# fritzsedlazeck/Sniffles

Hardware: NVIDIA H100
Metric: aligned long-read Gbp/s through lead->cluster->consensus (higher is better)
Workload: dtype int32

## Files before the change

### sniffles_b200/csrc/api.cu

```cuda
#include <algorithm>
#include <climits>
#include <cstdio>
#include <cstdlib>
#include <cstring>
#include <string>
#include <vector>
#include <dlfcn.h>
#include <omp.h>

#include "common.cuh"
#include "prims.cuh"
#include "extract.cuh"
#include "cluster.cuh"
#include "consensus.cuh"
#include "poa.cuh"
#include "combine.cuh"
#include "population.cuh"
#include "ingest.cuh"
#include "bgzf_write.cuh"
#include "genotype.cuh"
#include "rnames.cuh"
#include "reference.cuh"

template <bool Pinned> struct Buf {
// ... 786 lines not shown
    mark(ctx, "kept_bins");
    prims::exclusive_scan(ctx->launches, b.bin_nl, b.kl_off, b.scan_tmp, &ctr->n_bins, nb, &ctr->n_kl, st);
    prims::exclusive_scan(ctx->launches, b.bin_nlong, b.kll_off, b.scan_tmp, &ctr->n_bins, nb, &ctr->n_kll, st);
    prims::exclusive_scan(ctx->launches, b.bin_kept, b.kb_idx, b.scan_tmp, &ctr->n_bins, nb, &ctr->n_kbins, st);
    launch(ctx->launches, cluster::k_kbin_build, g, 128, 0, st, b);
    launch(ctx->launches, cluster::k_gather_kept, grid_for(nb, 256), 256, 0, st, b);
    mark(ctx, "merge_chains");
    launch(ctx->launches, cluster::k_seg_heads, g, 128, 0, st, b);
    prims::exclusive_scan(ctx->launches, b.flag, b.scan, b.scan_tmp, &ctr->n_kbins, nb, &ctr->n_segs, st);
    launch(ctx->launches, cluster::k_seg_build, g, 128, 0, st, b);
    launch(ctx->launches, cluster::k_merge, g, 128, 0, st, b);
    launch(ctx->launches, cluster::k_verify_cuts, g, 128, 0, st, b);
    prims::exclusive_scan(ctx->launches, b.flag, b.scan, b.scan_tmp, &ctr->n_kbins, nb, &ctr->n_clusters, st);
    launch(ctx->launches, cluster::k_cluster_build, g, 128, 0, st, b);
    mark(ctx, "cluster_call");
    CUDA_TRY(cudaEventRecord(ctx->ev_fork, st)); CUDA_TRY(cudaStreamWaitEvent(ctx->st_side, ctx->ev_fork, 0));
    launch(ctx->launches, cluster::k_cluster_block, NUM_SMS, cluster::CB_THREADS, cluster::CB_SMEM, ctx->st_side, b);
    launch(ctx->launches, cluster::k_cluster_warp<cluster::WARP_CAP, cluster::CWM_WARPS, true>, NUM_SMS * 2, cluster::CWM_WARPS * 32, cluster::CwCfg<cluster::WARP_CAP, cluster::CWM_WARPS>::smem, ctx->st_side, b);
    CUDA_TRY(cudaEventRecord(ctx->ev_join, ctx->st_side));
    launch(ctx->launches, cluster::k_cluster_warp<cluster::SMALL_CAP, cluster::CWS_WARPS, false>, NUM_SMS * 4, cluster::CWS_WARPS * 32, cluster::CwCfg<cluster::SMALL_CAP, cluster::CWS_WARPS>::smem, st, b);
    CUDA_TRY(cudaStreamWaitEvent(st, ctx->ev_join, 0));
    mark(ctx, "emit_cands");
    prims::exclusive_scan(ctx->launches, b.cl_nvalid, b.cl_cand_base, b.scan_tmp, &ctr->n_clusters, nb, &ctr->n_cand, st);
    prims::exclusive_scan(ctx->launches, b.cl_nlead, b.cl_lead_base, b.scan_tmp, &ctr->n_clusters, nb, &ctr->n_cand_leads, st);
    prims::exclusive_scan(ctx->launches, b.cl_nrn, b.cl_rn_base, b.scan_tmp, &ctr->n_clusters, nb, &ctr->n_rnames, st);
    launch(ctx->launches, cluster::k_emit_cands, NUM_SMS * 8, 128, 0, st, b);
    mark(ctx, "coverage");
    if (ctx->n_mask) launch(ctx->launches, cluster::k_mask_bp, grid_for((unsigned long long)ctx->n_mask * 32, 128), 128, 0, st, b, ctx->b_mask_task.as<uint32_t>(), ctx->n_mask, ctx->task_cov);
    launch(ctx->launches, cluster::k_coverage, NUM_SMS * 32, 128, 0, st, b);
    consensus::C& c = ctx->Cc;
    CUDA_TRY(cudaMemsetAsync(c.work, 0, sizeof(consensus::Work), st));
    mark(ctx, "consensus_plan");
    launch(ctx->launches, consensus::k_plan, grid_for(ctx->cap.cand, 128), 128, 0, st, c);
    prims::exclusive_scan(ctx->launches, c.alt_len, c.alt_off, b.scan_tmp, &ctr->n_cand, ctx->cap.cand, &ctr->n_alt_bytes, st);
    prims::exclusive_scan(ctx->launches, c.scr_len, c.scr_off, b.scan_tmp, &ctr->n_cand, ctx->cap.cand, &ctr->n_seq_bytes, st);
    prims::exclusive_scan_cols(ctx->launches, c.q_cnt, c.q_off, ctx->cap.cand + 1, consensus::NQ, ctx->q_scan_tmp, &ctr->n_cand, ctx->cap.cand, c.work->n, st);
    launch(ctx->launches, consensus::k_plan_finish, grid_for(ctx->cap.cand, 128), 128, 0, st, c);
    launch(ctx->launches, consensus::k_plan_slices, 1, 32, 0, st, c, ctx->n_slices);
    mark(ctx, nullptr);
    CUDA_TRY(cudaGetLastError());
    return 0;
}

static int enqueue_stage_c(snfb_ctx* ctx) {
    cluster::B& b = ctx->B; consensus::C& c = ctx->Cc; DevCounters* ctr = b.ctr; cudaStream_t st = ctx->st;
    c.seq = ctx->d_seq; c.arena_off = nullptr; ctx->seq_h2d_bytes = 0;
    if (ctx->seq_on_demand) {
        mark(ctx, "seq_requests");
        launch(ctx->launches, consensus::k_seq_requests, grid_for(ctx->cap.cand, 128), 128, 0, st, c, ctx->seq_req, ctx->cap.req, ctx->arena_off, &ctr->n_req, &ctr->n_req_units);
        mark(ctx, nullptr);
        CUDA_TRY(cudaMemcpyAsync(ctx->h_fin, ctr, sizeof(DevCounters), cudaMemcpyDeviceToHost, st));
        CUDA_TRY(cudaStreamSynchronize(st));
        const unsigned long long nreq = ctx->h_fin->n_req, nunits = ctx->h_fin->n_req_units;
        if (nreq <= ctx->cap.req && nunits <= ctx->cap.req16 && nreq) {
            if (ctx->h_seq_req.ensure(sizeof(consensus::SeqReq) * (nreq + 1)) || ctx->h_seq_arena.ensure(nunits * 16 + 64)) return fail(ctx, "out of pinned memory (seq arena)");
            CUDA_TRY(cudaMemcpyAsync(ctx->h_seq_req.p, ctx->seq_req, sizeof(consensus::SeqReq) * nreq, cudaMemcpyDeviceToHost, st));
            CUDA_TRY(cudaStreamSynchronize(st));
            const consensus::SeqReq* rq = ctx->h_seq_req.as<consensus::SeqReq>(); uint8_t* dst = ctx->h_seq_arena.as<uint8_t>(); const uint8_t* src = ctx->h_seq; const uint64_t nseq = ctx->n_seq;
            #pragma omp parallel for schedule(static, 256)
            for (long long i = 0; i < (long long)nreq; ++i) {
                unsigned long long s0 = rq[i].src; unsigned long long nbytes = rq[i].nbytes; if (s0 > nseq) s0 = nseq; if (s0 + nbytes > nseq) nbytes = nseq - s0;
                memcpy(dst + (size_t)rq[i].dst16 * 16, src + s0, (size_t)nbytes);
            }
            mark(ctx, "h2d_seq_slices", nunits * 16);
            CUDA_TRY(cudaMemcpyAsync(ctx->seq_arena, ctx->h_seq_arena.p, nunits * 16, cudaMemcpyHostToDevice, st));
            mark(ctx, nullptr);
            ctx->seq_h2d_bytes = nunits * 16;
        }
        c.seq = ctx->seq_arena; c.arena_off = ctx->arena_off;
    }
    CUDA_TRY(cudaEventRecord(ctx->ev_fork, st)); CUDA_TRY(cudaStreamWaitEvent(ctx->st_side, ctx->ev_fork, 0));
    for (int s = 0; s < ctx->n_slices; ++s) {
        cudaStream_t ss = (s & 1) ? ctx->st_side : st; const bool on_main = ss == st;
        if (s) CUDA_TRY(cudaStreamWaitEvent(ss, ctx->ev_aligned[s - 1], 0));
        if (on_main) mark(ctx, "consensus");
        launch(ctx->launches, consensus::k_prep, NUM_SMS * 8, 128, 0, ss, c, s);
        if (on_main) mark(ctx, "consensus_align");
        launch(ctx->launches, consensus::k_align, NUM_SMS * 7, consensus::ALIGN_WARPS * 32, 0, ss, c, s);
        CUDA_TRY(cudaEventRecord(ctx->ev_aligned[s], ss));
        if (on_main) mark(ctx, "consensus_vote");
        launch(ctx->launches, consensus::k_vote, NUM_SMS * 16, consensus::VOTE_THREADS, 0, ss, c, s);
        CUDA_TRY(cudaEventRecord(ctx->ev_slice[s], ss));
    }
    CUDA_TRY(cudaEventRecord(ctx->ev_join, ctx->st_side)); CUDA_TRY(cudaStreamWaitEvent(st, ctx->ev_join, 0));
    mark(ctx, nullptr);
    CUDA_TRY(cudaGetLastError());
    return 0;
}

static void initial_caps(snfb_ctx* ctx) {
    Caps& k = ctx->cap;
    const unsigned long long nrec = ctx->n_rec;
    const unsigned long long lead = std::max<unsigned long long>(1ull << 16, nrec) + (unsigned long long)extract::WALK_BLOCKS * (extract::WALK_THREADS / 32) * extract::WALK_SLOTS
                                    + (unsigned long long)extract::SA_BLOCKS * extract::SA_THREADS * extract::SLOT_CHUNK / 4;
    if (k.lead < lead) k.lead = lead;
    if (k.cand < k.lead / 8 + 1024) k.cand = k.lead / 8 + 1024;
    if (k.cand_lead < k.lead / 2 + 1024) k.cand_lead = k.lead / 2 + 1024;
    if (k.rn < k.lead / 2 + 1024) k.rn = k.lead / 2 + 1024;
    if (k.alt < (4ull << 20)) k.alt = 4ull << 20;
    if (k.scr16 < (2ull << 20)) k.scr16 = 2ull << 20;
    if (k.item < k.cand_lead / 2 + 1024) k.item = k.cand_lead / 2 + 1024;
    if (k.tile < k.cand + 4096) k.tile = k.cand + 4096;
    if (ctx->seq_on_demand) { if (k.req < k.cand_lead / 2 + 1024) k.req = k.cand_lead / 2 + 1024; if (k.req16 < (1ull << 20)) k.req16 = 1ull << 20; }
    else { if (k.req < 16) k.req = 16; if (k.req16 < 16) k.req16 = 16; }
}
static unsigned long long grown(unsigned long long need) { return need + need / 4 + 1024; }
static bool caps_fit(snfb_ctx* ctx, const DevCounters& c, const consensus::Work& work, int upto) {
// ... 821 lines not shown
```

### sniffles_b200/csrc/consensus.cuh

```cuda
#pragma once
#include "common.cuh"

namespace consensus {

constexpr int THREADS = 128;
constexpr int TAB = 2048;
constexpr uint8_t DASH = 0xff;
constexpr int MAXHIT = 512, MAXHIT_LIGHT = 384; constexpr uint32_t HEAVY_L = 3000;

enum { Q_BIG, Q_SMALL, Q_HEAVY, Q_LIGHT, Q_TILE, NQ };
constexpr int MAX_SLICES = 8, DEFAULT_SLICES = 2;
struct Slice { uint32_t c_lo, c_hi; uint32_t lo[NQ], hi[NQ]; unsigned long long alt_lo, alt_hi; };
struct Work {
    unsigned long long n[NQ];
    uint32_t pos[MAX_SLICES][4];
    Slice slice[MAX_SLICES];
};

struct C {
    const snfb_cand* cand; snfb_cand* cand_rw; const snfb_lead* cand_leads;
    const uint32_t* out_plo; const uint32_t* out_pn;
    const uint32_t* ord; const snfb_lead* kleads;
    const snfb_rec* rec; const uint8_t* seq;
    const uint32_t* arena_off;
    uint32_t* plan_best; uint32_t* plan_nother; uint32_t* plan_otot; uint32_t* alt_len; uint32_t* scr_len; uint32_t* alt_off; uint32_t* scr_off;
    uint8_t* alt; uint8_t* scr; unsigned long long alt_cap, scr_cap16, cand_cap;
    uint32_t* work_big; uint32_t* work_small; Work* work;
    uint32_t* q_cnt; uint32_t* q_off;
    struct Item { uint32_t cand; uint32_t k; uint32_t row; uint32_t rd_off; };
    Item* items_big; Item* items_small; uint2* tiles; unsigned long long item_cap, tile_cap;
    DevCounters* ctr; snfb_config cfg;
};

__device__ __forceinline__ uint8_t seq_code(const uint8_t* sq, long long q) { const uint8_t v = sq[q >> 1]; return (q & 1) ? (v & 15) : (v >> 4); }

__global__ void k_plan(C c) {
    const unsigned long long nc = c.ctr->n_cand < c.cand_cap ? c.ctr->n_cand : c.cand_cap;
    for (unsigned long long i = blockIdx.x * (unsigned long long)blockDim.x + threadIdx.x; i < nc; i += (unsigned long long)gridDim.x * blockDim.x) {
        uint32_t al = 0, sl = 0, heavy_n = 0, light_n = 0, tiles = 0; bool big = false;
        if (c.cand[i].svtype == SNFB_INS && !c.cfg.symbolic) {
            const snfb_cand* cd = &c.cand[i]; long nm = 0, bi = -1; long long bd = 0; long long tot = 0;
            for (int k = 0; k < cd->lead_n; ++k) { const snfb_lead* l = &c.cand_leads[cd->lead_off + k]; if (!(l->flags & SNFB_LF_HAS_SEQ)) continue;
                long long a = (long long)l->seq_len - cd->svlen; if (a < 0) a = -a; long long p = (long long)l->ref_start - cd->pos; if (p < 0) p = -p;
                const long long d = 2 * a + 3 * p; if (nm == 0 || d < bd) { bd = d; bi = k; } ++nm; tot += ((long long)l->seq_len + 7) & ~7ll; }
            if (nm > 0) {
                const uint32_t L = (uint32_t)c.cand_leads[cd->lead_off + bi].seq_len; al = L;
                const bool cons = (nm - 1 >= c.cfg.consensus_min_reads) && !c.cfg.no_consensus;
                c.plan_best[i] = (uint32_t)bi; c.plan_nother[i] = cons ? (uint32_t)(nm - 1) : 0u; c.plan_otot[i] = (uint32_t)(tot - ((L + 7u) & ~7u));
                const unsigned long long bytes = cons ? (unsigned long long)tot + 8 + (unsigned long long)(nm - 1) * ((L + 3u) & ~3u) + (unsigned long long)(nm - 1) * 16 + 64 + 16 + TAB * 8 : (unsigned long long)L + 24;
                sl = (uint32_t)((bytes + 15) / 16);
                c.cand_rw[i].alt_len = (int)L;
                big = (unsigned long long)L * (unsigned long long)nm > 60000ull;
                if (cons) { const bool heavy = L > HEAVY_L; heavy_n = heavy ? (uint32_t)(nm - 1) : 0u; light_n = heavy ? 0u : (uint32_t)(nm - 1); tiles = (L + 4095u) / 4096u; }
            }
        }
        c.alt_len[i] = al; c.scr_len[i] = sl;
        const size_t col = c.cand_cap + 1;
        c.q_cnt[Q_BIG * col + i] = sl && big; c.q_cnt[Q_SMALL * col + i] = sl && !big; c.q_cnt[Q_HEAVY * col + i] = heavy_n; c.q_cnt[Q_LIGHT * col + i] = light_n; c.q_cnt[Q_TILE * col + i] = tiles;
    }
}

__global__ void k_plan_finish(C c) {
    const unsigned long long nc = c.ctr->n_cand < c.cand_cap ? c.ctr->n_cand : c.cand_cap; const size_t col = c.cand_cap + 1;
    for (unsigned long long i = blockIdx.x * (unsigned long long)blockDim.x + threadIdx.x; i < nc; i += (unsigned long long)gridDim.x * blockDim.x) {
        if (!c.scr_len[i]) continue;
        c.cand_rw[i].alt_off = (int)c.alt_off[i];
        if (c.q_cnt[Q_BIG * col + i]) c.work_big[c.q_off[Q_BIG * col + i]] = (uint32_t)i; else c.work_small[c.q_off[Q_SMALL * col + i]] = (uint32_t)i;
        const uint32_t nh = c.q_cnt[Q_HEAVY * col + i], no = nh + c.q_cnt[Q_LIGHT * col + i];
        C::Item* dst = nh ? c.items_big : c.items_small; const uint32_t base = c.q_off[(nh ? Q_HEAVY : Q_LIGHT) * col + i];
        const snfb_cand* cd = &c.cand[i]; const uint32_t bi = c.plan_best[i];
        uint32_t row = 0, ro = 0;
        for (int k = 0; no && k < cd->lead_n; ++k) { const snfb_lead* l = &c.cand_leads[cd->lead_off + k]; if (!(l->flags & SNFB_LF_HAS_SEQ) || (uint32_t)k == bi) continue;
            if ((unsigned long long)base + row < c.item_cap) { C::Item it; it.cand = (uint32_t)i; it.k = (uint32_t)k; it.row = row; it.rd_off = ro; dst[base + row] = it; }
            ++row; ro += ((uint32_t)l->seq_len + 7u) & ~7u; }
        const uint32_t nt = c.q_cnt[Q_TILE * col + i], tb = c.q_off[Q_TILE * col + i];
        for (uint32_t t = 0; t < nt; ++t) if ((unsigned long long)tb + t < c.tile_cap) c.tiles[tb + t] = make_uint2((uint32_t)i, t);
    }
}

__global__ void k_plan_slices(C c, int k) {
    const int s = threadIdx.x; if (s >= k) return;
    const unsigned long long nc = c.ctr->n_cand < c.cand_cap ? c.ctr->n_cand : c.cand_cap; const size_t col = c.cand_cap + 1;
    const unsigned long long tot = c.ctr->n_seq_bytes;
    auto cut = [&](int j) -> uint32_t {
        if (j <= 0) return 0; if (j >= k) return (uint32_t)nc;
        const unsigned long long want = (tot * (unsigned long long)j + k - 1) / (unsigned long long)k;
        uint32_t lo = 0, hi = (uint32_t)nc;
        while (lo < hi) { const uint32_t m = (lo + hi) / 2; if (c.scr_off[m] < want) lo = m + 1; else hi = m; }
        return lo;
    };
    Slice sl; sl.c_lo = cut(s); sl.c_hi = cut(s + 1);
    for (int q = 0; q < NQ; ++q) { sl.lo[q] = sl.c_lo < nc ? c.q_off[q * col + sl.c_lo] : (uint32_t)c.work->n[q]; sl.hi[q] = sl.c_hi < nc ? c.q_off[q * col + sl.c_hi] : (uint32_t)c.work->n[q]; }
    sl.alt_lo = sl.c_lo < nc ? c.alt_off[sl.c_lo] : c.ctr->n_alt_bytes; sl.alt_hi = sl.c_hi < nc ? c.alt_off[sl.c_hi] : c.ctr->n_alt_bytes;
    c.work->slice[s] = sl;
}

__device__ __forceinline__ uint32_t nib_swap(uint32_t w) { return ((w & 0x0f0f0f0fu) << 4) | ((w >> 4) & 0x0f0f0f0fu); }
__device__ __forceinline__ uint32_t spread4(uint32_t x) { const uint32_t t = (x | (x << 8)) & 0x00ff00ffu; return (t | (t << 4)) & 0x0f0f0f0fu; }
__device__ __forceinline__ uint2 unpack8(const uint8_t* __restrict__ sq, long long q, int n) {
    const uintptr_t A = (uintptr_t)(sq + (q >> 1));
    const uint32_t* w = reinterpret_cast<const uint32_t*>(A & ~(uintptr_t)3);
    const int qn = (int)((A & 3) << 1) | (int)(q & 1);
    const uint32_t lo = nib_swap(__ldg(w)), hi = qn + n > 8 ? nib_swap(__ldg(w + 1)) : 0u;
    const uint32_t x = __funnelshift_r(lo, hi, 4 * qn);
    return make_uint2(spread4(x & 0xffffu), spread4(x >> 16));
}
__device__ __forceinline__ void unpack_span(const uint8_t* __restrict__ sq, long long off, int len, uint8_t* __restrict__ dst, int tid, int nthr) {
    const int full = ((uintptr_t)dst & 7) == 0 ? (len & ~7) : 0;
    int jb = tid * 8;
    for (; jb + 7 * nthr * 8 < full; jb += 8 * nthr * 8) {
        uint2 v[8];
        #pragma unroll
        for (int u = 0; u < 8; ++u) v[u] = unpack8(sq, off + jb + u * nthr * 8, 8);
        #pragma unroll
        for (int u = 0; u < 8; ++u) *reinterpret_cast<uint2*>(dst + jb + u * nthr * 8) = v[u];
    }
    for (; jb < full; jb += nthr * 8) *reinterpret_cast<uint2*>(dst + jb) = unpack8(sq, off + jb, 8);
    for (; jb < len; jb += nthr * 8) {
        const int n = min(8, len - jb); const uint2 v = unpack8(sq, off + jb, n);
        for (int t = 0; t < n; ++t) dst[jb + t] = (uint8_t)(((t < 4 ? v.x : v.y) >> (8 * (t & 3))) & 15u);
    }
}
__device__ inline void unpack_lead(const C& c, uint32_t cl_index, uint8_t* dst, int tid, int nthr) {
    const uint32_t plo = c.out_plo[cl_index], pn = c.out_pn[cl_index];
    long long o = 0;
    for (uint32_t p = 0; p < pn; ++p) {
        const uint32_t slot = c.ord[plo + p]; const snfb_lead* l = &c.kleads[slot];
        const uint8_t* sq = c.arena_off ? c.seq + (size_t)c.arena_off[slot] * 16 : c.seq + c.rec[l->rec].seq_off;
        unpack_span(sq, c.arena_off ? (l->seq_off & 1) : l->seq_off, l->seq_len, dst + o, tid, nthr);
        o += l->seq_len;
    }
}

__device__ __forceinline__ uint32_t kmer6(const uint8_t* s) { return (uint32_t)s[0] | ((uint32_t)s[1] << 4) | ((uint32_t)s[2] << 8) | ((uint32_t)s[3] << 12) | ((uint32_t)s[4] << 16) | ((uint32_t)s[5] << 20); }
__device__ __forceinline__ uint32_t kmer6_u(const uint8_t* s) {
    const uintptr_t A = (uintptr_t)s; const uint32_t* w = reinterpret_cast<const uint32_t*>(A & ~(uintptr_t)3); const uint32_t sh = (uint32_t)(A & 3) * 8;
    const uint32_t l0 = w[0], l1 = w[1], l2 = sh > 16 ? w[2] : 0u;
    const uint32_t x0 = __funnelshift_r(l0, l1, sh), x1 = __funnelshift_r(l1, l2, sh);
    uint32_t t = x0 & 0x0f0f0f0fu; t = (t | (t >> 4)) & 0x00ff00ffu; t = (t | (t >> 8)) & 0xffffu;
    return t | ((x1 & 15u) << 16) | (((x1 >> 8) & 15u) << 20);
}
__device__ __forceinline__ uint32_t kslot(uint32_t key) { return (key * 2654435761u) >> 21; }

struct SeqReq { unsigned long long src; uint32_t nbytes; uint32_t dst16; };
__global__ void k_seq_requests(C c, SeqReq* req, unsigned long long req_cap, uint32_t* arena_off_rw, unsigned long long* n_req, unsigned long long* n_units) {
    const unsigned long long nc = c.ctr->n_cand < c.cand_cap ? c.ctr->n_cand : c.cand_cap;
    for (unsigned long long i = blockIdx.x * (unsigned long long)blockDim.x + threadIdx.x; i < nc; i += (unsigned long long)gridDim.x * blockDim.x) {
        if (c.scr_len[i] == 0) continue;
        const snfb_cand* cd = &c.cand[i]; const bool cons = c.plan_nother[i] > 0;
        for (int k = 0; k < cd->lead_n; ++k) {
            const snfb_lead* cl = &c.cand_leads[cd->lead_off + k];
            if (!(cl->flags & SNFB_LF_HAS_SEQ) || (!cons && (uint32_t)k != c.plan_best[i])) continue;
            const uint32_t plo = c.out_plo[cd->lead_off + k], pn = c.out_pn[cd->lead_off + k];
            for (uint32_t p = 0; p < pn; ++p) {
                const uint32_t slot = c.ord[plo + p]; const snfb_lead* l = &c.kleads[slot];
                const unsigned long long b0 = (unsigned long long)l->seq_off >> 1, b1 = ((unsigned long long)l->seq_off + l->seq_len + 1) >> 1;
                const uint32_t nb = (uint32_t)(b1 - b0) + 1;
                const unsigned long long u = atomicAdd(n_units, (unsigned long long)((nb + 15) / 16));
                const unsigned long long r = atomicAdd(n_req, 1ULL);
                arena_off_rw[slot] = (uint32_t)u;
                if (r < req_cap) { req[r].src = c.rec[l->rec].seq_off + b0; req[r].nbytes = nb; req[r].dst16 = (uint32_t)u; }
            }
        }
    }
}



__device__ __forceinline__ int match_count(const uint8_t* a, const uint8_t* b, long n) {
    const uint32_t sa = ((uintptr_t)a & 3) * 8, sb = ((uintptr_t)b & 3) * 8;
    const uint32_t* wa = reinterpret_cast<const uint32_t*>((uintptr_t)a & ~(uintptr_t)3); const uint32_t* wb = reinterpret_cast<const uint32_t*>((uintptr_t)b & ~(uintptr_t)3);
    uint32_t alo = wa[0], blo = wb[0]; int mt = 0;
    long q = 0;
    #pragma unroll 2
    for (; q + 4 <= n; q += 4) {
        const uint32_t ahi = *++wa, bhi = *++wb;
        const uint32_t x = __funnelshift_r(alo, ahi, sa) ^ __funnelshift_r(blo, bhi, sb);
        mt += __popc(~(((x & 0x7f7f7f7fu) + 0x7f7f7f7fu) | x) & 0x80808080u);
        alo = ahi; blo = bhi;
    }
    if (q < n) {
        const uint32_t ahi = *++wa, bhi = *++wb;
        const uint32_t x = __funnelshift_r(alo, ahi, sa) ^ __funnelshift_r(blo, bhi, sb);
        mt += __popc(~(((x & 0x7f7f7f7fu) + 0x7f7f7f7fu) | x) & 0x80808080u & ((1u << (8 * (n - q))) - 1u));
    }
    return mt;
}
__device__ __forceinline__ void copy_bytes(uint8_t* dst, const uint8_t* src, long n) {
    long q = 0;
    while (q < n && ((uintptr_t)(dst + q) & 3)) { dst[q] = src[q]; ++q; }
    if (q + 4 <= n) {
        const uint8_t* s0 = src + q; const uint32_t sh = ((uintptr_t)s0 & 3) * 8;
        const uint32_t* ws = reinterpret_cast<const uint32_t*>((uintptr_t)s0 & ~(uintptr_t)3); uint32_t lo = ws[0];
        uint32_t* wd = reinterpret_cast<uint32_t*>(dst + q);
        #pragma unroll 4
        for (; q + 4 <= n; q += 4) { const uint32_t hi = *++ws; *wd++ = __funnelshift_r(lo, hi, sh); lo = hi; }
    }
    for (; q < n; ++q) dst[q] = src[q];
}
__device__ __forceinline__ void fill_dash(uint8_t* dst, long n) {
    long q = 0;
    while (q < n && ((uintptr_t)(dst + q) & 3)) dst[q++] = DASH;
    for (; q + 4 <= n; q += 4) *reinterpret_cast<uint32_t*>(dst + q) = 0xffffffffu;
    for (; q < n; ++q) dst[q] = DASH;
}

__device__ __forceinline__ uint32_t load_u32_unaligned(const uint8_t* p) {
    const uintptr_t A = (uintptr_t)p; const uint32_t* w = reinterpret_cast<const uint32_t*>(A & ~(uintptr_t)3);
    return __funnelshift_r(w[0], w[1], (uint32_t)(A & 3) * 8);
}
template <int G>
__device__ __forceinline__ int group_match(const uint8_t* a, const uint8_t* b, long n, int sub) {
    int mt = 0;
    #pragma unroll 2
    for (long q = 4L * sub; q < n; q += 4L * G) {
        const uint32_t x = load_u32_unaligned(a + q) ^ load_u32_unaligned(b + q);
        uint32_t eq = ~(((x & 0x7f7f7f7fu) + 0x7f7f7f7fu) | x) & 0x80808080u;
        if (n - q < 4) eq &= (1u << (8 * (n - q))) - 1u;
        mt += __popc(eq);
    }
    return mt;
}
template <int G> __device__ __forceinline__ int group_sum(int v) {
    #pragma unroll
    for (int o = G / 2; o > 0; o >>= 1) v += __shfl_xor_sync(FULL, v, o);
    return v;
}
struct WarpGrp {
    static constexpr int NTHR = 32; int tid;
    __device__ __forceinline__ void sync() const { __syncwarp(); }
    __device__ __forceinline__ int excl(int v, int& tot) const {
        int inc = v;
        #pragma unroll
        for (int o = 1; o < 32; o <<= 1) { const int t = __shfl_up_sync(FULL, inc, o); if (tid >= o) inc += t; }
        tot = __shfl_sync(FULL, inc, 31); return inc - v;
    }
    __device__ __forceinline__ int exclmax(int v, int& tot) const {
        int inc = v;
        #pragma unroll
        for (int o = 1; o < 32; o <<= 1) { const int t = __shfl_up_sync(FULL, inc, o); if (tid >= o) inc = max(inc, t); }
        tot = __shfl_sync(FULL, inc, 31); int e = __shfl_up_sync(FULL, inc, 1); if (tid == 0) e = -1; return e;
    }
    __device__ __forceinline__ long sum(long v) const { return (long)__reduce_add_sync(FULL, (unsigned)v); }
};
template <int WARPS>
struct BlockGrp {
    static constexpr int NTHR = WARPS * 32; int tid; int* red;
    __device__ __forceinline__ void sync() const { __syncthreads(); }
    __device__ __forceinline__ int excl(int v, int& tot) const {
        const int lane = tid & 31, w = tid >> 5; int inc = v;
        #pragma unroll
        for (int o = 1; o < 32; o <<= 1) { const int t = __shfl_up_sync(FULL, inc, o); if (lane >= o) inc += t; }
        if (lane == 31) red[w] = inc;
        __syncthreads();
        int base = 0, all = 0;
        #pragma unroll
        for (int k = 0; k < WARPS; ++k) { const int t = red[k]; if (k < w) base += t; all += t; }
        __syncthreads();
        tot = all; return base + inc - v;
    }
    __device__ __forceinline__ int exclmax(int v, int& tot) const {
        const int lane = tid & 31, w = tid >> 5; int inc = v;
        #pragma unroll
        for (int o = 1; o < 32; o <<= 1) { const int t = __shfl_up_sync(FULL, inc, o); if (lane >= o) inc = max(inc, t); }
        int e = __shfl_up_sync(FULL, inc, 1); if (lane == 0) e = -1;
        if (lane == 31) red[w] = inc;
        __syncthreads();
        int all = -1;
        #pragma unroll
        for (int k = 0; k < WARPS; ++k) { const int t = red[k]; if (k < w) e = max(e, t); all = max(all, t); }
        __syncthreads();
        tot = all; return e;
    }
    __device__ __forceinline__ long sum(long v) const {
        const int lane = tid & 31, w = tid >> 5; const int sv = (int)__reduce_add_sync(FULL, (unsigned)v);
        if (lane == 0) red[w] = sv;
        __syncthreads();
        int all = 0;
        #pragma unroll
        for (int k = 0; k < WARPS; ++k) all += red[k];
        __syncthreads();
        return (long)all;
    }
};

template <int G>
__device__ __forceinline__ long segments_pass(const int* hi, const int* hj, int* hcl, int na, long c0, long j0, long L, const uint8_t* rd, const uint8_t* best, int tid, int nthr) {
    const int PER = nthr / G; const int grp = tid / G, sub = tid % G; long span = 0;
    for (int mb = 1; mb < na; mb += PER) {
        const int m = mb + grp; const bool v = m < na;
        long li = 0, lj = 0, i = 0, j = 0; if (v) { li = hi[m - 1]; lj = hj[m - 1]; i = hi[m]; j = hj[m]; }
        long cs = c0 + lj - j0; if (cs > L) cs = L;
        const long d = j - lj; long fwd_j = d; if (cs + fwd_j > L) fwd_j = L - cs;
        const bool el = v && i - li == fwd_j && fwd_j > 0;
        long nc = 0; if (el) { nc = L - 1 - li; if (nc > d) nc = d; if (nc < 0) nc = 0; }
        const int mt = group_sum<G>(group_match<G>(rd + lj + 1, best + li + 1, nc, sub));
        int st = -1; bool second = false;
        if (el) { if (sub == 0) span += d; if (__ddiv_rn((double)mt, (double)d) >= 0.5) { if (cs == li && fwd_j == d && nc == d) st = mt; else second = true; } }
        const int m2 = group_sum<G>(group_match<G>(rd + lj, best + cs, second ? fwd_j : 0, sub));
        if (second) st = m2;
        if (v && sub == 0) hcl[m] = st;
    }
    return span;
}

struct Layout { uint8_t* best; uint8_t* oth; uint8_t* rows; uint8_t* acc; uint32_t Ls; };
__device__ __forceinline__ Layout cand_layout(const C& c, uint32_t ci, uint32_t L, uint32_t no) {
    Layout y; y.best = c.scr + (size_t)c.scr_off[ci] * 16; y.oth = y.best + ((L + 7u) & ~7u);
    y.rows = reinterpret_cast<uint8_t*>(((uintptr_t)(y.oth + c.plan_otot[ci]) + 3) & ~(uintptr_t)3); y.Ls = (L + 3u) & ~3u; y.acc = y.rows + (size_t)no * y.Ls;
    return y;
}
__device__ __forceinline__ uint8_t* cand_table(const C& c, uint32_t ci, uint32_t** keys, int** pos) {
    uint8_t* scr = c.scr + (size_t)c.scr_off[ci] * 16;
    uint8_t* end = scr + (size_t)c.scr_len[ci] * 16;
    *keys = reinterpret_cast<uint32_t*>(end - TAB * 8); *pos = reinterpret_cast<int*>(end - TAB * 4);
    return scr;
}

__global__ void __launch_bounds__(128) k_prep(C c, int s) {
    __shared__ uint32_t s_cand;
    static const char CODE[17] = "=ACMGRSVTWYHKDBN";
    const Slice& sl = c.work->slice[s];
    for (;;) {
        __syncthreads();
        if (threadIdx.x == 0) { const uint32_t q = atomicAdd(&c.work->pos[s][0], 1u); const uint32_t nb = sl.hi[Q_BIG] - sl.lo[Q_BIG], ns = sl.hi[Q_SMALL] - sl.lo[Q_SMALL];
            s_cand = q < nb ? c.work_big[sl.lo[Q_BIG] + q] : (q < nb + ns ? c.work_small[sl.lo[Q_SMALL] + q - nb] : 0xffffffffu); }
        __syncthreads();
        const uint32_t ci = s_cand; if (ci == 0xffffffffu) break;
        const uint32_t L = c.alt_len[ci];
        if ((unsigned long long)c.alt_off[ci] + L > c.alt_cap || (unsigned long long)c.scr_off[ci] + c.scr_len[ci] > c.scr_cap16) { if (threadIdx.x == 0) atomicAdd(&c.ctr->scratch_overflow, 1ULL); continue; }
        const snfb_cand cd = c.cand[ci];
        uint32_t* tk; int* tp; uint8_t* best = cand_table(c, ci, &tk, &tp);
        unpack_lead(c, cd.lead_off + c.plan_best[ci], best, threadIdx.x, blockDim.x);
        const uint32_t no = c.plan_nother[ci];
        if (no == 0 || L == 0) { __syncthreads(); uint8_t* out = c.alt + c.alt_off[ci]; for (uint32_t h = threadIdx.x; h < L; h += blockDim.x) out[h] = (uint8_t)CODE[best[h]]; continue; }
        for (int i = threadIdx.x; i < TAB; i += blockDim.x) { tk[i] = 0xffffffffu; tp[i] = -1; }
        __syncthreads();
        const long skip = c.cfg.consensus_kmer_skip_base + (long)__dmul_rn((double)L, c.cfg.consensus_kmer_skip_seqlen_mult);
        for (long i = (long)threadIdx.x * skip; i < (long)L - 6; i += (long)blockDim.x * skip) {
            const uint32_t key = kmer6_u(best + i); uint32_t s = kslot(key);
            for (;;) { const uint32_t old = atomicCAS(&tk[s], 0xffffffffu, key); if (old == 0xffffffffu || old == key) break; s = (s + 1) & (TAB - 1); }
            if (atomicCAS(&tp[s], -1, (int)i) != -1) tp[s] = -2;
        }
    }
}

template <typename G>
__device__ __forceinline__ void align_item(const C& c, const C::Item it, const G g, int* hi, int* hj, int* hcl, int* run_st, int* run_len, int cap) {
    const int tid = g.tid; constexpr int NT = G::NTHR; const int klen = 6;
    const uint32_t ci = it.cand; const uint32_t L = c.alt_len[ci];
    if ((unsigned long long)c.scr_off[ci] + c.scr_len[ci] > c.scr_cap16) return;
    const snfb_cand* cd = &c.cand[ci];
    uint32_t* t_key; int* t_pos; cand_table(c, ci, &t_key, &t_pos);
    const uint32_t no = c.plan_nother[ci];
    const Layout y = cand_layout(c, ci, L, no);
    uint8_t* best = y.best; uint8_t* acc = y.acc;
    const snfb_lead* l = &c.cand_leads[cd->lead_off + it.k];
    const long Lo = l->seq_len; uint8_t* rd = y.oth + it.rd_off; uint8_t* row = y.rows + (size_t)it.row * y.Ls;
    const long skip = c.cfg.consensus_kmer_skip_base + (long)__dmul_rn((double)L, c.cfg.consensus_kmer_skip_seqlen_mult);
    unpack_lead(c, cd->lead_off + it.k, rd, tid, NT);
    g.sync();
    int nh = 0;
    const long nk = Lo - klen > 0 ? (Lo - klen + skip - 1) / skip : 0;
    for (long kb = 0; kb < nk; kb += 4 * NT) {
        uint32_t key[4], sl[4], tk[4]; int ai[4];
        #pragma unroll
        for (int u = 0; u < 4; ++u) { const long kk = kb + u * NT + tid; key[u] = kk < nk ? kmer6_u(rd + kk * skip) : 0u; sl[u] = kslot(key[u]); }
        #pragma unroll
        for (int u = 0; u < 4; ++u) tk[u] = kb + u * NT + tid < nk ? t_key[sl[u]] : 0xffffffffu;
        #pragma unroll
        for (int u = 0; u < 4; ++u) while (tk[u] != 0xffffffffu && tk[u] != key[u]) { sl[u] = (sl[u] + 1) & (TAB - 1); tk[u] = t_key[sl[u]]; }
        #pragma unroll
        for (int u = 0; u < 4; ++u) ai[u] = tk[u] != 0xffffffffu ? t_pos[sl[u]] : -1;
        #pragma unroll
        for (int u = 0; u < 4; ++u) {
            if (kb + (long)u * NT >= nk) break;
            const long j = (kb + u * NT + tid) * skip;
            if (ai[u] >= 0) { long d = ai[u] - j; if (d < 0) d = -d; if (d > klen) ai[u] = -1; }
            int tot; const int off = g.excl(ai[u] >= 0 ? 1 : 0, tot);
            if (ai[u] >= 0) { const int p = nh + off; if (p < cap) { hi[p] = ai[u]; hj[p] = (int)j; } }
            nh += tot;
        }
    }
    if (nh > cap) nh = cap;
    g.sync();
    int na = 0, pm = -1;
    for (int hb = 0; hb < nh; hb += NT) {
        const int h = hb + tid; const int vi = h < nh ? hi[h] : -1, vj = h < nh ? hj[h] : 0;
        int tmax; const int exc = max(g.exclmax(vi, tmax), pm);
        const bool accp = h < nh && vi > exc;
        int tot; const int off = g.excl(accp ? 1 : 0, tot);
        g.sync();
        if (accp) { hi[na + off] = vi; hj[na + off] = vj; }
        na += tot; pm = max(pm, tmax);
        g.sync();
    }
    const long j0 = na ? hj[0] : 0, c0 = (na && j0 > 0) ? hi[0] : 0;
    long span = skip > 12 ? segments_pass<8>(hi, hj, hcl, na, c0, j0, (long)L, rd, best, tid, NT) : segments_pass<1>(hi, hj, hcl, na, c0, j0, (long)L, rd, best, tid, NT);
    span = g.sum(span);
    g.sync();
    {
        int* hr = hi;
        for (int m = tid; m < na; m += NT) { run_st[m] = 0; run_len[m] = 0; }
        g.sync();
        int run_base = 0;
        for (int mb = 1; mb < na; mb += NT) {
            const int m = mb + tid; int st = -1; long len = 0;
            if (m < na) { const long lj = hj[m - 1]; long cs = c0 + lj - j0; if (cs > (long)L) cs = (long)L; len = hj[m] - lj; if (cs + len > (long)L) len = (long)L - cs; st = hcl[m]; }
            int tot; const int rid = run_base + g.excl((m < na && st < 0 && len > 0) ? 1 : 0, tot);
            g.sync();
            if (m < na) { hr[m] = rid; if (st >= 0) { atomicAdd(&run_st[rid], st); atomicAdd(&run_len[rid], (int)len); } }
            run_base += tot;
        }
        g.sync();
        for (int m = 1 + tid; m < na; m += NT) {
            if (hcl[m] < 0) continue;
            const int r = hr[m], ident = run_st[r];
            if (!(__ddiv_rn((double)ident, (double)run_len[r]) > 0.5 && ident > 5)) hcl[m] = -1;
        }
        g.sync();
    }
    {
        long cl = 0; if (na) { cl = c0 + hj[na - 1] - j0; if (cl > (long)L) cl = (long)L; }
        const uint8_t* src0 = rd + (j0 - c0);
        #pragma unroll 4
        for (long X = 4L * tid; X < (long)L; X += 4L * NT) {
            uint32_t v = 0xffffffffu;
            if (X + 4 > c0 && X < cl) {
                v = load_u32_unaligned(src0 + X);
                if (X < c0) v |= (1u << (8 * (c0 - X))) - 1u;
                if (X + 4 > cl) v |= ~((1u << (8 * (cl - X))) - 1u);
            }
            *reinterpret_cast<uint32_t*>(row + X) = v;
        }
        g.sync();
        for (int m = 1 + tid; m < na; m += NT) {
            if (hcl[m] >= 0) continue;
            const long lj = hj[m - 1]; long cs = c0 + lj - j0; if (cs > (long)L) cs = (long)L;
            long len = hj[m] - lj; if (cs + len > (long)L) len = (long)L - cs;
            if (len > 0) fill_dash(row + cs, len);
        }
    }
    if (tid == 0) acc[it.row] = __ddiv_rn((double)span, (double)L) > 0.2;
    g.sync();
}

constexpr int ALIGN_WARPS = 4;
__global__ void __launch_bounds__(ALIGN_WARPS * 32, 7) k_align(C c, int s) {
    __shared__ int sm[5][ALIGN_WARPS * MAXHIT_LIGHT]; __shared__ int s_red[2 * ALIGN_WARPS]; __shared__ uint32_t s_q;
    static_assert(ALIGN_WARPS * MAXHIT_LIGHT >= MAXHIT, "a block item needs MAXHIT entries");
    const int lane = lane_id(), warp = threadIdx.x >> 5;
    const Slice& sl = c.work->slice[s];
    const uint32_t b0 = sl.lo[Q_HEAVY], nb = (uint32_t)min((unsigned long long)sl.hi[Q_HEAVY], c.item_cap), s0 = sl.lo[Q_LIGHT], ns = (uint32_t)min((unsigned long long)sl.hi[Q_LIGHT], c.item_cap);
    for (;;) {
        __syncthreads();
        if (threadIdx.x == 0) s_q = b0 + atomicAdd(&c.work->pos[s][1], 1u);
        __syncthreads();
        const uint32_t q = s_q; if (q >= nb) break;
        BlockGrp<ALIGN_WARPS> g; g.tid = threadIdx.x; g.red = s_red;
        align_item(c, c.items_big[q], g, sm[0], sm[1], sm[2], sm[3], sm[4], ALIGN_WARPS * MAXHIT_LIGHT);
    }
    __syncthreads();
    for (;;) {
        uint32_t q = 0; if (lane == 0) q = s0 + atomicAdd(&c.work->pos[s][2], 1u);
        q = __shfl_sync(FULL, q, 0);
        if (q >= ns) break;
        WarpGrp g; g.tid = lane; const int o = warp * MAXHIT_LIGHT;
        align_item(c, c.items_small[q], g, sm[0] + o, sm[1] + o, sm[2] + o, sm[3] + o, sm[4] + o, MAXHIT_LIGHT);
    }
}

constexpr int VOTE_LIST = 256;
__device__ __forceinline__ void vote_add(unsigned long long (&cnt)[4], uint32_t code) {
    const unsigned long long inc = 1ull << (16 * (code & 3u)); const uint32_t sel = (code >> 2) & 3u;
    #pragma unroll
    for (int k = 0; k < 4; ++k) cnt[k] += sel == (uint32_t)k ? inc : 0ull;
}
constexpr int VOTE_THREADS = 64;
__global__ void __launch_bounds__(VOTE_THREADS) k_vote(C c, int s) {
    __shared__ uint2 s_tile; __shared__ int s_nacc, s_nlist; __shared__ uint16_t s_rows[VOTE_LIST];
    static const char CODE[17] = "=ACMGRSVTWYHKDBN";
    const Slice& sl = c.work->slice[s];
    for (;;) {
        __syncthreads();
        if (threadIdx.x == 0) { const uint32_t q = sl.lo[Q_TILE] + atomicAdd(&c.work->pos[s][3], 1u); s_tile = q < sl.hi[Q_TILE] && q < c.tile_cap ? c.tiles[q] : make_uint2(0xffffffffu, 0); }
        __syncthreads();
// ... 90 lines not shown
```

Baseline: 9857.

## Align consensus reads on packed 4-bit nibbles instead of unpacked bytes

After: 10290, median of 6. 1.04x the previous value.

```diff
diff --git a/sniffles_b200/csrc/api.cu b/sniffles_b200/csrc/api.cu
--- a/sniffles_b200/csrc/api.cu
+++ b/sniffles_b200/csrc/api.cu
@@ -862,7 +862,8 @@
         CUDA_TRY(cudaMemcpyAsync(ctx->h_fin, ctr, sizeof(DevCounters), cudaMemcpyDeviceToHost, st));
         CUDA_TRY(cudaStreamSynchronize(st));
         const unsigned long long nreq = ctx->h_fin->n_req, nunits = ctx->h_fin->n_req_units;
-        if (nreq <= ctx->cap.req && nunits <= ctx->cap.req16 && nreq) {
+        if (nreq > ctx->cap.req || nunits > ctx->cap.req16) return 0;
+        if (nreq) {
             if (ctx->h_seq_req.ensure(sizeof(consensus::SeqReq) * (nreq + 1)) || ctx->h_seq_arena.ensure(nunits * 16 + 64)) return fail(ctx, "out of pinned memory (seq arena)");
             CUDA_TRY(cudaMemcpyAsync(ctx->h_seq_req.p, ctx->seq_req, sizeof(consensus::SeqReq) * nreq, cudaMemcpyDeviceToHost, st));
             CUDA_TRY(cudaStreamSynchronize(st));
diff --git a/sniffles_b200/csrc/consensus.cuh b/sniffles_b200/csrc/consensus.cuh
--- a/sniffles_b200/csrc/consensus.cuh
+++ b/sniffles_b200/csrc/consensus.cuh
@@ -33,21 +33,23 @@
 };
 
 __device__ __forceinline__ uint8_t seq_code(const uint8_t* sq, long long q) { const uint8_t v = sq[q >> 1]; return (q & 1) ? (v & 15) : (v >> 4); }
+__device__ __forceinline__ uint32_t packed_bytes(uint32_t len) { return ((len + 15u) & ~15u) / 2u; }
 
 __global__ void k_plan(C c) {
     const unsigned long long nc = c.ctr->n_cand < c.cand_cap ? c.ctr->n_cand : c.cand_cap;
     for (unsigned long long i = blockIdx.x * (unsigned long long)blockDim.x + threadIdx.x; i < nc; i += (unsigned long long)gridDim.x * blockDim.x) {
         uint32_t al = 0, sl = 0, heavy_n = 0, light_n = 0, tiles = 0; bool big = false;
         if (c.cand[i].svtype == SNFB_INS && !c.cfg.symbolic) {
-            const snfb_cand* cd = &c.cand[i]; long nm = 0, bi = -1; long long bd = 0; long long tot = 0;
+            const snfb_cand* cd = &c.cand[i]; long nm = 0, bi = -1; long long bd = 0; long long tot = 0, bpk = 0;
             for (int k = 0; k < cd->lead_n; ++k) { const snfb_lead* l = &c.cand_leads[cd->lead_off + k]; if (!(l->flags & SNFB_LF_HAS_SEQ)) continue;
                 long long a = (long long)l->seq_len - cd->svlen; if (a < 0) a = -a; long long p = (long long)l->ref_start - cd->pos; if (p < 0) p = -p;
-                const long long d = 2 * a + 3 * p; if (nm == 0 || d < bd) { bd = d; bi = k; } ++nm; tot += ((long long)l->seq_len + 7) & ~7ll; }
+                const long long d = 2 * a + 3 * p; if (nm == 0 || d < bd) { bd = d; bi = k; } ++nm;
+                const long long pk = c.out_pn[cd->lead_off + k] != 1 ? packed_bytes((uint32_t)l->seq_len) : 0; tot += pk; if (bi == k) bpk = pk; }
             if (nm > 0) {
                 const uint32_t L = (uint32_t)c.cand_leads[cd->lead_off + bi].seq_len; al = L;
                 const bool cons = (nm - 1 >= c.cfg.consensus_min_reads) && !c.cfg.no_consensus;
-                c.plan_best[i] = (uint32_t)bi; c.plan_nother[i] = cons ? (uint32_t)(nm - 1) : 0u; c.plan_otot[i] = (uint32_t)(tot - ((L + 7u) & ~7u));
-                const unsigned long long bytes = cons ? (unsigned long long)tot + 8 + (unsigned long long)(nm - 1) * ((L + 3u) & ~3u) + (unsigned long long)(nm - 1) * 16 + 64 + 16 + TAB * 8 : (unsigned long long)L + 24;
+                c.plan_best[i] = (uint32_t)bi; c.plan_nother[i] = cons ? (uint32_t)(nm - 1) : 0u; c.plan_otot[i] = (uint32_t)(tot - bpk);
+                const unsigned long long bytes = cons ? (unsigned long long)((L + 7u) & ~7u) + packed_bytes(L) + (unsigned long long)(tot - bpk) + 8 + (unsigned long long)(nm - 1) * ((L + 3u) & ~3u) + (unsigned long long)(nm - 1) * 16 + 64 + 16 + TAB * 8 : (unsigned long long)L + 24;
                 sl = (uint32_t)((bytes + 15) / 16);
                 c.cand_rw[i].alt_len = (int)L;
                 big = (unsigned long long)L * (unsigned long long)nm > 60000ull;
@@ -72,7 +74,7 @@
         uint32_t row = 0, ro = 0;
         for (int k = 0; no && k < cd->lead_n; ++k) { const snfb_lead* l = &c.cand_leads[cd->lead_off + k]; if (!(l->flags & SNFB_LF_HAS_SEQ) || (uint32_t)k == bi) continue;
             if ((unsigned long long)base + row < c.item_cap) { C::Item it; it.cand = (uint32_t)i; it.k = (uint32_t)k; it.row = row; it.rd_off = ro; dst[base + row] = it; }
-            ++row; ro += ((uint32_t)l->seq_len + 7u) & ~7u; }
+            ++row; if (c.out_pn[cd->lead_off + k] != 1) ro += packed_bytes((uint32_t)l->seq_len); }
         const uint32_t nt = c.q_cnt[Q_TILE * col + i], tb = c.q_off[Q_TILE * col + i];
         for (uint32_t t = 0; t < nt; ++t) if ((unsigned long long)tb + t < c.tile_cap) c.tiles[tb + t] = make_uint2((uint32_t)i, t);
     }
@@ -97,12 +99,27 @@
 
 __device__ __forceinline__ uint32_t nib_swap(uint32_t w) { return ((w & 0x0f0f0f0fu) << 4) | ((w >> 4) & 0x0f0f0f0fu); }
 __device__ __forceinline__ uint32_t spread4(uint32_t x) { const uint32_t t = (x | (x << 8)) & 0x00ff00ffu; return (t | (t << 4)) & 0x0f0f0f0fu; }
+struct Nib {
+    const uint32_t* w; int o;
+    __device__ static __forceinline__ Nib at(const uint8_t* p, long long q) {
+        const uintptr_t A = (uintptr_t)(p + (q >> 1));
+        Nib r; r.w = reinterpret_cast<const uint32_t*>(A & ~(uintptr_t)3); r.o = (int)((A & 3) << 1) | (int)(q & 1); return r;
+    }
+    template <bool SWAP = true> __device__ __forceinline__ uint32_t get8(int q, int n) const {
+        const int b = o + q; const uint32_t* x = w + (b >> 3); const int qn = b & 7;
+        const uint32_t lo = SWAP ? nib_swap(x[0]) : x[0], hi = qn + n > 8 ? (SWAP ? nib_swap(x[1]) : x[1]) : 0u;
+        return __funnelshift_r(lo, hi, 4 * qn);
+    }
+    __device__ __forceinline__ uint32_t take(int r, int m, int n) const {
+        const int a = r < 0 ? 0 : r, e = r + m < n ? r + m : n;
+        if (e <= a) return 0u;
+        const int k = e - a; uint32_t x = get8(a, k);
+        if (k < 8) x &= (1u << (4 * k)) - 1u;
+        return x << (4 * (a - r));
+    }
+};
 __device__ __forceinline__ uint2 unpack8(const uint8_t* __restrict__ sq, long long q, int n) {
-    const uintptr_t A = (uintptr_t)(sq + (q >> 1));
-    const uint32_t* w = reinterpret_cast<const uint32_t*>(A & ~(uintptr_t)3);
-    const int qn = (int)((A & 3) << 1) | (int)(q & 1);
-    const uint32_t lo = nib_swap(__ldg(w)), hi = qn + n > 8 ? nib_swap(__ldg(w + 1)) : 0u;
-    const uint32_t x = __funnelshift_r(lo, hi, 4 * qn);
+    const uint32_t x = Nib::at(sq, q).get8(0, n);
     return make_uint2(spread4(x & 0xffffu), spread4(x >> 16));
 }
 __device__ __forceinline__ void unpack_span(const uint8_t* __restrict__ sq, long long off, int len, uint8_t* __restrict__ dst, int tid, int nthr) {
@@ -120,6 +137,10 @@
         const int n = min(8, len - jb); const uint2 v = unpack8(sq, off + jb, n);
         for (int t = 0; t < n; ++t) dst[jb + t] = (uint8_t)(((t < 4 ? v.x : v.y) >> (8 * (t & 3))) & 15u);
     }
+}
+__device__ __forceinline__ Nib lead_bases(const C& c, uint32_t slot) {
+    const snfb_lead* l = &c.kleads[slot];
+    return c.arena_off ? Nib::at(c.seq + (size_t)c.arena_off[slot] * 16, l->seq_off & 1) : Nib::at(c.seq + c.rec[l->rec].seq_off, l->seq_off);
 }
 __device__ inline void unpack_lead(const C& c, uint32_t cl_index, uint8_t* dst, int tid, int nthr) {
     const uint32_t plo = c.out_plo[cl_index], pn = c.out_pn[cl_index];
@@ -131,6 +152,29 @@
         o += l->seq_len;
     }
 }
+__device__ inline void pack_lead(const C& c, uint32_t cl_index, long len, uint32_t* dst, int tid, int nthr, bool arena_order) {
+    const uint32_t plo = c.out_plo[cl_index], pn = c.out_pn[cl_index];
+    const long nw = (long)(packed_bytes((uint32_t)len) / 4);
+    uint32_t p = 0; int o = 0, n = 0; Nib b{};
+    if (pn) { const uint32_t slot = c.ord[plo]; b = lead_bases(c, slot); n = c.kleads[slot].seq_len; }
+    for (long w = tid; w < nw; w += nthr) {
+        const int q = 8 * (int)w; uint32_t x = 0;
+        if (pn) {
+            while (o + n <= q && p + 1 < pn) { o += n; ++p; const uint32_t slot = c.ord[plo + p]; b = lead_bases(c, slot); n = c.kleads[slot].seq_len; }
+            x = b.take(q - o, 8, n);
+            int o2 = o + n;
+            for (uint32_t p2 = p + 1; p2 < pn && o2 < q + 8; ++p2) {
+                const uint32_t slot = c.ord[plo + p2]; const int n2 = c.kleads[slot].seq_len;
+                x |= lead_bases(c, slot).take(q - o2, 8, n2); o2 += n2;
+            }
+        }
+        dst[w] = arena_order ? nib_swap(x) : x;
+    }
+}
+__device__ __forceinline__ Nib lead_reader(const C& c, uint32_t cl_index, const uint8_t* copy) {
+    if (c.out_pn[cl_index] == 1) return lead_bases(c, c.ord[c.out_plo[cl_index]]);
+    Nib r; r.w = reinterpret_cast<const uint32_t*>(copy); r.o = 0; return r;
+}
 
 __device__ __forceinline__ uint32_t kmer6(const uint8_t* s) { return (uint32_t)s[0] | ((uint32_t)s[1] << 4) | ((uint32_t)s[2] << 8) | ((uint32_t)s[3] << 12) | ((uint32_t)s[4] << 16) | ((uint32_t)s[5] << 20); }
 __device__ __forceinline__ uint32_t kmer6_u(const uint8_t* s) {
@@ -140,6 +184,7 @@
     uint32_t t = x0 & 0x0f0f0f0fu; t = (t | (t >> 4)) & 0x00ff00ffu; t = (t | (t >> 8)) & 0xffffu;
     return t | ((x1 & 15u) << 16) | (((x1 >> 8) & 15u) << 20);
 }
+__device__ __forceinline__ uint32_t kmer6_n(const Nib& s, int q) { return s.get8(q, 6) & 0xffffffu; }
 __device__ __forceinline__ uint32_t kslot(uint32_t key) { return (key * 2654435761u) >> 21; }
 
 struct SeqReq { unsigned long long src; uint32_t nbytes; uint32_t dst16; };
@@ -167,37 +212,6 @@
 
 
 
-__device__ __forceinline__ int match_count(const uint8_t* a, const uint8_t* b, long n) {
-    const uint32_t sa = ((uintptr_t)a & 3) * 8, sb = ((uintptr_t)b & 3) * 8;
-    const uint32_t* wa = reinterpret_cast<const uint32_t*>((uintptr_t)a & ~(uintptr_t)3); const uint32_t* wb = reinterpret_cast<const uint32_t*>((uintptr_t)b & ~(uintptr_t)3);
-    uint32_t alo = wa[0], blo = wb[0]; int mt = 0;
-    long q = 0;
-    #pragma unroll 2
-    for (; q + 4 <= n; q += 4) {
-        const uint32_t ahi = *++wa, bhi = *++wb;
-        const uint32_t x = __funnelshift_r(alo, ahi, sa) ^ __funnelshift_r(blo, bhi, sb);
-        mt += __popc(~(((x & 0x7f7f7f7fu) + 0x7f7f7f7fu) | x) & 0x80808080u);
-        alo = ahi; blo = bhi;
-    }
-    if (q < n) {
-        const uint32_t ahi = *++wa, bhi = *++wb;
-        const uint32_t x = __funnelshift_r(alo, ahi, sa) ^ __funnelshift_r(blo, bhi, sb);
-        mt += __popc(~(((x & 0x7f7f7f7fu) + 0x7f7f7f7fu) | x) & 0x80808080u & ((1u << (8 * (n - q))) - 1u));
-    }
-    return mt;
-}
-__device__ __forceinline__ void copy_bytes(uint8_t* dst, const uint8_t* src, long n) {
-    long q = 0;
-    while (q < n && ((uintptr_t)(dst + q) & 3)) { dst[q] = src[q]; ++q; }
-    if (q + 4 <= n) {
-        const uint8_t* s0 = src + q; const uint32_t sh = ((uintptr_t)s0 & 3) * 8;
-        const uint32_t* ws = reinterpret_cast<const uint32_t*>((uintptr_t)s0 & ~(uintptr_t)3); uint32_t lo = ws[0];
-        uint32_t* wd = reinterpret_cast<uint32_t*>(dst + q);
-        #pragma unroll 4
-        for (; q + 4 <= n; q += 4) { const uint32_t hi = *++ws; *wd++ = __funnelshift_r(lo, hi, sh); lo = hi; }
-    }
-    for (; q < n; ++q) dst[q] = src[q];
-}
 __device__ __forceinline__ void fill_dash(uint8_t* dst, long n) {
     long q = 0;
     while (q < n && ((uintptr_t)(dst + q) & 3)) dst[q++] = DASH;
@@ -205,18 +219,15 @@
     for (; q < n; ++q) dst[q] = DASH;
 }
 
-__device__ __forceinline__ uint32_t load_u32_unaligned(const uint8_t* p) {
-    const uintptr_t A = (uintptr_t)p; const uint32_t* w = reinterpret_cast<const uint32_t*>(A & ~(uintptr_t)3);
-    return __funnelshift_r(w[0], w[1], (uint32_t)(A & 3) * 8);
-}
 template <int G>
-__device__ __forceinline__ int group_match(const uint8_t* a, const uint8_t* b, long n, int sub) {
+__device__ __forceinline__ int group_match(const Nib& a, long ia, const Nib& b, long ib, long n, int sub) {
     int mt = 0;
-    #pragma unroll 2
-    for (long q = 4L * sub; q < n; q += 4L * G) {
-        const uint32_t x = load_u32_unaligned(a + q) ^ load_u32_unaligned(b + q);
-        uint32_t eq = ~(((x & 0x7f7f7f7fu) + 0x7f7f7f7fu) | x) & 0x80808080u;
-        if (n - q < 4) eq &= (1u << (8 * (n - q))) - 1u;
+    for (long q = 8L * sub; q < n; q += 8L * G) {
+        const int k = n - q < 8 ? (int)(n - q) : 8;
+        uint32_t x = a.get8((int)(ia + q), k) ^ b.get8<false>((int)(ib + q), k);
+        x |= x >> 1; x |= x >> 2;
+        uint32_t eq = ~x & 0x11111111u;
+        if (k < 8) eq &= (1u << (4 * k)) - 1u;
         mt += __popc(eq);
     }
     return mt;
@@ -285,7 +296,7 @@
 };
 
 template <int G>
-__device__ __forceinline__ long segments_pass(const int* hi, const int* hj, int* hcl, int na, long c0, long j0, long L, const uint8_t* rd, const uint8_t* best, int tid, int nthr) {
+__device__ __forceinline__ long segments_pass(const int* hi, const int* hj, int* hcl, int na, long c0, long j0, long L, const Nib& rd, const Nib& best, int tid, int nthr) {
     const int PER = nthr / G; const int grp = tid / G, sub = tid % G; long span = 0;
     for (int mb = 1; mb < na; mb += PER) {
         const int m = mb + grp; const bool v = m < na;
@@ -294,19 +305,19 @@
         const long d = j - lj; long fwd_j = d; if (cs + fwd_j > L) fwd_j = L - cs;
         const bool el = v && i - li == fwd_j && fwd_j > 0;
         long nc = 0; if (el) { nc = L - 1 - li; if (nc > d) nc = d; if (nc < 0) nc = 0; }
-        const int mt = group_sum<G>(group_match<G>(rd + lj + 1, best + li + 1, nc, sub));
+        const int mt = group_sum<G>(group_match<G>(rd, lj + 1, best, li + 1, nc, sub));
         int st = -1; bool second = false;
         if (el) { if (sub == 0) span += d; if (__ddiv_rn((double)mt, (double)d) >= 0.5) { if (cs == li && fwd_j == d && nc == d) st = mt; else second = true; } }
-        const int m2 = group_sum<G>(group_match<G>(rd + lj, best + cs, second ? fwd_j : 0, sub));
+        const int m2 = group_sum<G>(group_match<G>(rd, lj, best, cs, second ? fwd_j : 0, sub));
         if (second) st = m2;
         if (v && sub == 0) hcl[m] = st;
     }
     return span;
 }
 
-struct Layout { uint8_t* best; uint8_t* oth; uint8_t* rows; uint8_t* acc; uint32_t Ls; };
+struct Layout { uint8_t* best; uint8_t* best4; uint8_t* oth; uint8_t* rows; uint8_t* acc; uint32_t Ls; };
 __device__ __forceinline__ Layout cand_layout(const C& c, uint32_t ci, uint32_t L, uint32_t no) {
-    Layout y; y.best = c.scr + (size_t)c.scr_off[ci] * 16; y.oth = y.best + ((L + 7u) & ~7u);
+    Layout y; y.best = c.scr + (size_t)c.scr_off[ci] * 16; y.best4 = y.best + ((L + 7u) & ~7u); y.oth = y.best4 + packed_bytes(L);
     y.rows = reinterpret_cast<uint8_t*>(((uintptr_t)(y.oth + c.plan_otot[ci]) + 3) & ~(uintptr_t)3); y.Ls = (L + 3u) & ~3u; y.acc = y.rows + (size_t)no * y.Ls;
     return y;
 }
@@ -334,6 +345,7 @@
         unpack_lead(c, cd.lead_off + c.plan_best[ci], best, threadIdx.x, blockDim.x);
         const uint32_t no = c.plan_nother[ci];
         if (no == 0 || L == 0) { __syncthreads(); uint8_t* out = c.alt + c.alt_off[ci]; for (uint32_t h = threadIdx.x; h < L; h += blockDim.x) out[h] = (uint8_t)CODE[best[h]]; continue; }
+        pack_lead(c, cd.lead_off + c.plan_best[ci], L, reinterpret_cast<uint32_t*>(best + ((L + 7u) & ~7u)), threadIdx.x, blockDim.x, false);
         for (int i = threadIdx.x; i < TAB; i += blockDim.x) { tk[i] = 0xffffffffu; tp[i] = -1; }
         __syncthreads();
         const long skip = c.cfg.consensus_kmer_skip_base + (long)__dmul_rn((double)L, c.cfg.consensus_kmer_skip_seqlen_mult);
@@ -354,18 +366,18 @@
     uint32_t* t_key; int* t_pos; cand_table(c, ci, &t_key, &t_pos);
     const uint32_t no = c.plan_nother[ci];
     const Layout y = cand_layout(c, ci, L, no);
-    uint8_t* best = y.best; uint8_t* acc = y.acc;
+    uint8_t* acc = y.acc; const Nib best = Nib::at(y.best4, 0);
     const snfb_lead* l = &c.cand_leads[cd->lead_off + it.k];
-    const long Lo = l->seq_len; uint8_t* rd = y.oth + it.rd_off; uint8_t* row = y.rows + (size_t)it.row * y.Ls;
+    const long Lo = l->seq_len; uint8_t* row = y.rows + (size_t)it.row * y.Ls;
     const long skip = c.cfg.consensus_kmer_skip_base + (long)__dmul_rn((double)L, c.cfg.consensus_kmer_skip_seqlen_mult);
-    unpack_lead(c, cd->lead_off + it.k, rd, tid, NT);
-    g.sync();
+    const Nib rd = lead_reader(c, cd->lead_off + it.k, y.oth + it.rd_off);
+    if (c.out_pn[cd->lead_off + it.k] != 1) { pack_lead(c, cd->lead_off + it.k, Lo, reinterpret_cast<uint32_t*>(y.oth + it.rd_off), tid, NT, true); g.sync(); }
     int nh = 0;
     const long nk = Lo - klen > 0 ? (Lo - klen + skip - 1) / skip : 0;
     for (long kb = 0; kb < nk; kb += 4 * NT) {
         uint32_t key[4], sl[4], tk[4]; int ai[4];
         #pragma unroll
-        for (int u = 0; u < 4; ++u) { const long kk = kb + u * NT + tid; key[u] = kk < nk ? kmer6_u(rd + kk * skip) : 0u; sl[u] = kslot(key[u]); }
+        for (int u = 0; u < 4; ++u) { const long kk = kb + u * NT + tid; key[u] = kk < nk ? kmer6_n(rd, (int)(kk * skip)) : 0u; sl[u] = kslot(key[u]); }
         #pragma unroll
         for (int u = 0; u < 4; ++u) tk[u] = kb + u * NT + tid < nk ? t_key[sl[u]] : 0xffffffffu;
         #pragma unroll
@@ -396,7 +408,7 @@
         g.sync();
     }
     const long j0 = na ? hj[0] : 0, c0 = (na && j0 > 0) ? hi[0] : 0;
-    long span = skip > 12 ? segments_pass<8>(hi, hj, hcl, na, c0, j0, (long)L, rd, best, tid, NT) : segments_pass<1>(hi, hj, hcl, na, c0, j0, (long)L, rd, best, tid, NT);
+    long span = skip > 12 ? segments_pass<4>(hi, hj, hcl, na, c0, j0, (long)L, rd, best, tid, NT) : segments_pass<1>(hi, hj, hcl, na, c0, j0, (long)L, rd, best, tid, NT);
     span = g.sum(span);
     g.sync();
     {
@@ -422,16 +434,17 @@
     }
     {
         long cl = 0; if (na) { cl = c0 + hj[na - 1] - j0; if (cl > (long)L) cl = (long)L; }
-        const uint8_t* src0 = rd + (j0 - c0);
-        #pragma unroll 4
-        for (long X = 4L * tid; X < (long)L; X += 4L * NT) {
-            uint32_t v = 0xffffffffu;
-            if (X + 4 > c0 && X < cl) {
-                v = load_u32_unaligned(src0 + X);
-                if (X < c0) v |= (1u << (8 * (c0 - X))) - 1u;
-                if (X + 4 > cl) v |= ~((1u << (8 * (cl - X))) - 1u);
-            }
-            *reinterpret_cast<uint32_t*>(row + X) = v;
+        for (long X = 8L * tid; X < (long)L; X += 8L * NT) {
+            unsigned long long v = ~0ull;
+            if (X + 8 > c0 && X < cl) {
+                const int q = (int)(X + j0 - c0);
+                const uint32_t x = q >= 0 && q + 8 <= (int)Lo ? rd.get8(q, 8) : rd.take(q, 8, (int)Lo);
+                v = (unsigned long long)spread4(x & 0xffffu) | ((unsigned long long)spread4(x >> 16) << 32);
+                if (X < c0) v |= (1ull << (8 * (c0 - X))) - 1ull;
+                if (X + 8 > cl) v |= ~((1ull << (8 * (cl - X))) - 1ull);
+            }
+            *reinterpret_cast<uint32_t*>(row + X) = (uint32_t)v;
+            if (X + 4 < (long)L) *reinterpret_cast<uint32_t*>(row + X + 4) = (uint32_t)(v >> 32);
         }
         g.sync();
         for (int m = 1 + tid; m < na; m += NT) {
```
